# zubair-irshad/HunyuanWorld-Mirror

Hardware: AMD Instinct MI355X
Metric: views/sec (higher is better)
Workload: dtype bf16; 1 GPU; 8-view 518x518 bf16, no priors, camera+depth+pointmap+normal heads, 8 views/GPU, full 1.23B-param arch; views_per_gpu=8, global_views=8, parallelism=view-shard x1, collective=none (1 GPU)

## Files before the change

### hunyuanworld-mirror_amd/_lib.py

```python
from __future__ import annotations

import ctypes as C
import os

import torch

_HERE = os.path.dirname(os.path.abspath(__file__))
LIB_PATH = os.environ.get("WM_HIP_LIB") or os.path.join(_HERE, "libwm_hip.so")

WM_DT = {"bf16": 0, "f16": 1, "fp16": 1, "float16": 1, "bfloat16": 0}
EPI_F32, EPI_T16, EPI_GELU_T16, EPI_RESID = 0, 1, 2, 3


class wm_config(C.Structure):
    _fields_ = [
        ("img_size", C.c_int32), ("patch_size", C.c_int32), ("embed_dim", C.c_int32), ("gs_dim", C.c_int32),
        ("enable_cond", C.c_int32), ("enable_cam", C.c_int32), ("enable_pts", C.c_int32), ("enable_depth", C.c_int32),
        ("enable_norm", C.c_int32), ("enable_gs", C.c_int32),
        ("depth", C.c_int32), ("num_heads", C.c_int32), ("mlp_ratio", C.c_int32), ("num_register_tokens", C.c_int32),
        ("intermediate_idxs", C.c_int32 * 4),
        ("rope_freq", C.c_float),
        ("dino_depth", C.c_int32), ("dino_heads", C.c_int32),
        ("cam_trunk_depth", C.c_int32), ("cam_heads", C.c_int32), ("cam_steps", C.c_int32),
        ("dpt_features", C.c_int32),
# ... 2 lines not shown
    ]


_FP = C.c_void_p


class wm_outputs(C.Structure):
    _fields_ = [(n, _FP) for n in (
        "camera_params", "camera_poses", "camera_intrs", "depth", "depth_conf", "pts3d", "pts3d_conf",
        "normals", "normals_conf", "gs_depth", "gs_depth_conf", "splat_means", "splat_quats", "splat_scales",
        "splat_opacities", "splat_sh", "splat_weights")] + [("taps", _FP * 4)]


class wm_raster_options(C.Structure):
    _fields_ = [("antialiased", C.c_int), ("depth_mode", C.c_int), ("eps2d", C.c_float), ("near_plane", C.c_float), ("far_plane", C.c_float),
                ("radius_clip", C.c_float), ("backgrounds", C.c_void_p)]


EXPORTS = [
    "wm_create", "wm_destroy", "wm_last_error", "wm_set_weight", "wm_finalize_weights", "wm_host_resample_pos",
    "wm_workspace_bytes", "wm_reserve", "wm_set_workspace", "wm_missing_name", "wm_share_weights", "wm_forward", "wm_forward_sharded", "wm_rccl_unique_id", "wm_comm_init_rccl",
    "wm_local_group_create", "wm_local_group_destroy", "wm_comm_init_local", "wm_allgather", "wm_profile_enable", "wm_profile_read",
    "wm_op_gemm", "wm_op_gemm_resid_ln", "wm_op_gemm_qkv", "wm_op_attention", "wm_op_layernorm", "wm_op_qkv_post", "wm_op_conv", "wm_op_bilinear",
    "wm_op_linear_f32", "wm_host_to_16", "wm_set_tuning", "wm_op_attention_split", "wm_op_attention_ex", "wm_op_attention_flag_count", "wm_op_gs_splat", "wm_op_conv3x3_up", "wm_depth_to_world", "wm_confidence_mask", "wm_confidence_mask_workspace_bytes", "wm_preprocess_image", "wm_preprocess_image_size",
    "wm_preprocess_image_workspace_bytes", "wm_rasterize_splats", "wm_rasterize_workspace_bytes", "wm_rasterize_splats_backward", "wm_rasterize_backward_workspace_bytes", "wm_prune_gs", "wm_prune_gs_workspace_bytes", "wm_op_up_conv_n32", "wm_op_conv3x3_gemm16", "wm_op_conv_ex", "wm_op_upconv3x3_tap", "wm_op_tconv", "wm_op_upconv_gather",
    "wm_depth_edge", "wm_normals_edge", "wm_point_filter_mask_workspace_bytes", "wm_point_filter_mask",
    "wm_op_im2col", "wm_op_im2col7", "wm_op_dino_tokens", "wm_op_vgt_special", "wm_op_gemm_rowmap", "wm_op_gemm_convt", "wm_op_layernorm_rows",
    "wm_op_bilinear_add", "wm_op_bilinear16", "wm_op_copy2d", "wm_op_small_attention", "wm_op_adaln", "wm_op_cam_update", "wm_op_cam_matrices",
    "wm_op_linear_f32_ex", "wm_op_dpt_tail", "wm_op_up_conv_n32_tail", "wm_op_dpt_tap_front",
    "wm_photometric_loss_workspace_bytes", "wm_photometric_loss_forward_workspace_bytes", "wm_photometric_loss", "wm_photometric_loss_backward",
    "wm_rasterize_backward_workspace_bytes_ex", "wm_rasterize_splats_backward_ex", "wm_rasterize_means2d",
    "wm_rasterize_backward_workspace_bytes_cam", "wm_rasterize_splats_backward_cam",
    "wm_rasterize_splats_sh", "wm_rasterize_backward_workspace_bytes_sh", "wm_rasterize_splats_backward_sh",
    "wm_rasterize_splats_opt", "wm_rasterize_backward_workspace_bytes_opt", "wm_rasterize_splats_backward_opt",
    "wm_densify_accumulate", "wm_densify_plan_workspace_bytes", "wm_densify_plan", "wm_densify_gather",
    "wm_mcmc_inject_noise", "wm_mcmc_partition_workspace_bytes", "wm_mcmc_partition", "wm_mcmc_relocation", "wm_mcmc_scatter", "wm_mcmc_zero_rows",
    "wm_bilagrid_slice", "wm_bilagrid_slice_backward_workspace_bytes", "wm_bilagrid_slice_backward", "wm_bilagrid_tv_workspace_bytes",
    "wm_bilagrid_tv", "wm_bilagrid_tv_backward",
    "wm_appearance_forward", "wm_appearance_backward_workspace_bytes", "wm_appearance_backward",
    "wm_depth_loss_workspace_bytes", "wm_depth_loss", "wm_depth_loss_backward", "wm_project_depth_points",
]

_lib = None


def lib() -> C.CDLL:
    global _lib
# ... 22 lines not shown
    L.wm_missing_name.argtypes = [vp, i32]
    L.wm_missing_name.restype = C.c_char_p
    L.wm_forward.argtypes = [vp, vp, i32, i32, i32, vp, vp, vp, C.POINTER(C.c_int32), C.POINTER(wm_outputs), vp]
    L.wm_forward_sharded.argtypes = [vp, vp, i32, i32, i32, i32, i32, vp, vp, vp, C.POINTER(C.c_int32),
                                     C.POINTER(wm_outputs), vp]
    L.wm_rccl_unique_id.argtypes = [vp]
    L.wm_comm_init_rccl.argtypes = [vp, vp, i32, i32]
    L.wm_local_group_create.argtypes = [i32]
    L.wm_local_group_create.restype = vp
    L.wm_local_group_destroy.argtypes = [vp]
    L.wm_local_group_destroy.restype = None
    L.wm_comm_init_local.argtypes = [vp, vp, i32]
    L.wm_allgather.argtypes = [vp, vp, vp, C.c_size_t, vp]
    L.wm_profile_enable.argtypes = [vp, i32]
    L.wm_profile_read.argtypes = [vp, i32, C.POINTER(C.c_double), C.POINTER(C.c_int64)]
    L.wm_op_gemm.argtypes = [i32, i32, vp, vp, vp, vp, vp, i32, i32, i32, vp]
    L.wm_op_gemm_resid_ln.argtypes = [i32, vp, vp, vp, vp, vp, vp, vp, f32, vp, vp, vp, i32, i32, i32, C.POINTER(i32), vp]
    L.wm_op_gemm_qkv.argtypes = [i32, vp, vp, vp, vp, vp, vp, vp, vp, vp, vp, vp, vp, i32, i32, i32, i32, i32, i32, f32, vp]
    L.wm_op_attention.argtypes = [i32, vp, vp, vp, vp, i32, i32, i32, i32, i32, vp]
    L.wm_op_attention_split.argtypes = [i32, vp, vp, vp, vp, i32, i32, i32, i32, i32, i32, vp, vp, vp]
    L.wm_op_attention_ex.argtypes = [i32, vp, vp, vp, vp, i32, i32, i32, i32, i32, i32, vp, vp, vp, vp]
    L.wm_op_attention_flag_count.argtypes = [i32, i32, i32]
    L.wm_op_attention_flag_count.restype = C.c_size_t
    L.wm_op_layernorm.argtypes = [vp, vp, vp, vp, i32, i32, f32, i32, i32, vp]
    L.wm_op_qkv_post.argtypes = [i32, vp, vp, vp, vp, vp, vp, vp, vp, vp, vp, i32, i32, i32, i32, i32, f32, vp]
    L.wm_op_conv.argtypes = [i32, vp, vp, vp, vp, vp, vp, i32, i32, i32, i32, i32, i32, i32, i32, i32, i32, vp]
    L.wm_op_bilinear.argtypes = [vp, vp, i32, i32, i32, i32, i32, i32, vp]
    L.wm_op_linear_f32.argtypes = [vp, vp, vp, vp, i32, i32, i32, i32, i32, i32, vp]
    L.wm_host_to_16.argtypes = [vp, vp, C.c_size_t, i32]
    L.wm_host_to_16.restype = None
    L.wm_depth_to_world.argtypes = [vp, vp, vp, vp, vp, vp, i32, i32, i32, f32, vp]
    L.wm_depth_to_world.restype = i32
    L.wm_confidence_mask_workspace_bytes.argtypes = [C.c_size_t]
    L.wm_confidence_mask_workspace_bytes.restype = C.c_size_t
    L.wm_confidence_mask.argtypes = [vp, C.c_size_t, f32, vp, vp, C.c_size_t, vp]
    L.wm_confidence_mask.restype = i32
    L.wm_depth_edge.argtypes = [vp, vp, i32, i32, i32, i32, i32, f32, i32, f32, vp, vp]
    L.wm_depth_edge.restype = i32
    L.wm_normals_edge.argtypes = [vp, vp, i32, i32, i32, i32, C.c_double, vp, vp]
    L.wm_normals_edge.restype = i32
    L.wm_point_filter_mask_workspace_bytes.argtypes = [i32, i32, i32]
    L.wm_point_filter_mask_workspace_bytes.restype = C.c_size_t
    L.wm_point_filter_mask.argtypes = [vp, vp, vp, i32, i32, i32, i32, C.c_double, i32, C.c_double, f32, vp, vp, vp, C.c_size_t, vp]
    L.wm_point_filter_mask.restype = i32
    L.wm_op_up_conv_n32.argtypes = [i32, vp, vp, vp, vp, i32, i32, i32, i32, i32, i32, vp, vp, i32, vp, vp]
    L.wm_op_up_conv_n32.restype = i32
# ... 162 lines not shown
```

### hunyuanworld-mirror_amd/csrc/attention.hip

```cpp
#include "wm_common.h"
#include "wm_kernels.h"

namespace {

__device__ __forceinline__ void wm_dma16(const void* g, uint32_t lds_dst) {
  uint32_t keep;
  asm volatile("s_mov_b32 %0, m0\n\ts_mov_b32 m0, %2\n\ts_nop 0\n\tglobal_load_lds_dwordx4 %1, off\n\ts_mov_b32 m0, %0"
               : "=&s"(keep) : "v"(g), "s"(lds_dst) : "memory");
}

constexpr int KVB = 64;
constexpr int TILE_B = KVB * 64 * 2;
constexpr float LOG2E = 1.4426950408889634f;

typedef __attribute__((address_space(3))) s16x4* lds_s16x4p;

typedef __attribute__((ext_vector_type(2))) float f32x2;
typedef __attribute__((ext_vector_type(2))) __bf16 bf16x2;
typedef __attribute__((ext_vector_type(2))) _Float16 f16x2;
__device__ __forceinline__ uint32_t pack2(float a, float b, int T) {
  const f32x2 v = {a, b};
  return T == WM_T_BF16 ? __builtin_bit_cast(uint32_t, __builtin_convertvector(v, bf16x2))
                        : __builtin_bit_cast(uint32_t, __builtin_convertvector(v, f16x2));
}
// ... 559 lines not shown
    M = fmaxf(M, ml.x);
  }
  float L = 0.f;
  float4 o = make_float4(0, 0, 0, 0);
  for (int s = 0; s < p.kv_splits; ++s) {
    const float w = __builtin_amdgcn_exp2f(m[s] - M);
    L += w * l[s];
    const float4 v = *(const float4*)(p.part_o + ((size_t)s * p.q_rows + row) * (p.H * 64) + head * 64 + d4 * 4);
    o.x += w * v.x; o.y += w * v.y; o.z += w * v.z; o.w += w * v.w;
  }
  const float inv = 1.0f / L;
  uint2 u;
  u.x = pack2(o.x * inv, o.y * inv, T);
  u.y = pack2(o.z * inv, o.w * inv, T);
  *(uint2*)((u16*)p.O + (row * p.H + head) * 64 + d4 * 4) = u;
}

template <int T, int NW, int QB, int MINW, int LZ = 1, int STG = 1>
hipError_t launch(const WmAttnArgs& a_in, hipStream_t s, int fast = 0) {
  const bool use_v3 = fast != 0;
  constexpr int QT = NW * 32 * QB;
  WmAttnArgs a = a_in;
  a.only_if = nullptr;
  const int tiles_per_seq = (a.seq_len + QT - 1) / QT;
  const int nseq = a.q_rows / a.seq_len;
  {
    static const int ncu = [] { hipDeviceProp_t pr; int d = 0; (void)hipGetDevice(&d); return hipGetDeviceProperties(&pr, d) == hipSuccess ? pr.multiProcessorCount : 256; }();
    const long slots = (long)ncu * MINW * 4 / NW, blocks = (long)tiles_per_seq * nseq * a.H;
    const int seg_rows = a.kv_chunks > 1 ? a.kv_rows_per_chunk : a.seq_len;
    const int ntiles = (seg_rows + KVB - 1) / KVB * a.kv_chunks;
    int lim = a.part_o && a.part_ml ? (a.max_splits > 0 ? a.max_splits : WM_ATTN_MAX_SPLITS) : 1;
    lim = lim < WM_ATTN_MAX_SPLITS ? lim : WM_ATTN_MAX_SPLITS;
    lim = lim < ntiles / 8 ? lim : (ntiles / 8 > 1 ? ntiles / 8 : 1);
    int best = 1;
    const int forced_splits = wm_tune(WM_TUNE_ATTN_SPLITS, 0);
    const int tail_mode = wm_tune(WM_TUNE_ATTN_TAIL, 1);
    if (a.kv_splits > 0) best = a.kv_splits < lim ? a.kv_splits : lim;
    else if (forced_splits > 0) best = forced_splits < lim ? forced_splits : lim;
    else if (a.kv_chunks > 1 && lim >= 2) best = lim < 4 ? lim : 4;
    if (a.force_partial) best = a_in.kv_splits > 0 ? (a_in.kv_splits < lim ? a_in.kv_splits : lim) : 1;
    a.kv_splits = best;
    a.full_units = 0;
    const long tail = blocks % slots;
    if (!a.force_partial && a_in.kv_splits == 0 && forced_splits <= 0 && lim >= 2 && ntiles >= (use_v3 ? 16 : 64) && blocks > slots && tail > 0 && tail_mode != 0) {
      auto round_cost = [&](long n) { const long rem = n % slots; return (double)(n / slots) + (rem == 0 ? 0.0 : (rem * 2 <= slots && fast != 4) ? 0.73 : 1.0); };
      double best_cost = round_cost(tail);
      int bs = 1;
      for (int S = 2; S <= lim; ++S) {
        const double c = round_cost(tail * S) / S + 0.01 * S;
        if (c < best_cost - 0.05) { best_cost = c; bs = S; }
      }
      if (tail_mode > 1) bs = tail_mode < lim ? tail_mode : lim;
      if (bs > 1) { a.kv_splits = bs; a.full_units = (int)(blocks - tail); }
      else if (best > 1) a.kv_splits = best;
    }
  }
  const int units = tiles_per_seq * nseq * a.H;
  const int nfull = a.kv_splits > 1 ? a.full_units : units;
  dim3 grid(nfull + (units - nfull) * a.kv_splits), block(NW * 64);
  if (use_v3) {
    hipError_t e = fast == 4 ? wm_launch_attention_v4(a, (int)grid.x, a.unit_flags, s) : wm_launch_attention_v3(a, (int)grid.x, a.unit_flags, s);
    if (e != hipSuccess) return e;
    a.only_if = a.unit_flags;
  }
#ifdef WM_ATTN_TIMING_EXPERIMENT
  const int dbg_skip = wm_tune(WM_TUNE_ATTN_DEBUG_SKIP, 0);
#else
  constexpr int dbg_skip = 0;
#endif
  if (!(use_v3 && (dbg_skip & 1))) hipLaunchKernelGGL((attn_fwd_kernel<T, NW, QB, MINW, LZ, STG>), grid, block, 0, s, a);
  if (a.kv_splits > 1 && !a.force_partial && !(dbg_skip & 2))
    hipLaunchKernelGGL((attn_combine_kernel<T>), dim3((unsigned)((units - nfull) * (QT / 16))), dim3(256), 0, s, a, QT);
  return hipGetLastError();
}

}

hipError_t wm_launch_attention_combine(const WmAttnArgs& a_in, int slots, hipStream_t s) {
  if (a_in.q_rows <= 0) return hipSuccess;
  if (slots < 1 || slots > WM_ATTN_MAX_SPLITS || !a_in.part_o || !a_in.part_ml) return hipErrorInvalidValue;
  constexpr int QT = 256;
  WmAttnArgs a = a_in;
  a.kv_splits = slots;
  a.full_units = 0;
  const int units = ((a.seq_len + QT - 1) / QT) * (a.q_rows / a.seq_len) * a.H;
  if (a.dtype == WM_T_BF16) hipLaunchKernelGGL((attn_combine_kernel<WM_T_BF16>), dim3((unsigned)(units * (QT / 16))), dim3(256), 0, s, a, QT);
  else hipLaunchKernelGGL((attn_combine_kernel<WM_T_F16>), dim3((unsigned)(units * (QT / 16))), dim3(256), 0, s, a, QT);
  return hipGetLastError();
}

int wm_attention_variant(const WmAttnArgs& a) {
  const int forced = wm_tune(WM_TUNE_ATTN_QB, 0);
  const int seg_rows = a.kv_chunks > 1 ? a.kv_rows_per_chunk : a.seq_len;
  const bool fast_ok = a.unit_flags != nullptr && seg_rows >= 512;
  const bool v3ok = a.dtype == WM_T_BF16 && fast_ok;
  int qb = forced ? forced : 8;
  if (!forced && a.kv_chunks == 1 && a.seq_len <= 2048) qb = (a.dtype == WM_T_BF16 && a.q_rows / a.seq_len >= 16) ? 7 : 4;
  if ((qb == 7 && !v3ok) || (qb == 8 && !fast_ok) || qb == 0) qb = (a.kv_chunks == 1 && a.seq_len <= 2048) ? 4 : 3;
  if (a.force_partial && qb != 7 && qb != 8 && qb != 3) qb = forced ? -1 : 3;
  return qb;
}
void wm_attention_geometry(const WmAttnArgs& a, int* unit_rows, int* blocks_per_cu) {
  const int qb = wm_attention_variant(a);
  *unit_rows = qb == 8 ? 512 : qb == 4 || qb == 11 ? 128 : 256;
  *blocks_per_cu = qb == 8 ? 1 : qb == 4 || qb == 11 ? 3 : 2;
}

hipError_t wm_launch_attention(const WmAttnArgs& a, hipStream_t s) {
  if (a.q_rows <= 0) return hipSuccess;
  if (a.seq_len <= 0 || a.q_rows % a.seq_len != 0 || a.kv_chunks < 1) return hipErrorInvalidValue;
  const int qb = wm_attention_variant(a);
  if (qb < 0) return hipErrorInvalidValue;
  const int seg_rows = a.kv_chunks > 1 ? a.kv_rows_per_chunk : a.seq_len;
  if (qb == 7) return launch<WM_T_BF16, 4, 2, 2>(a, s, 3);
  if (qb == 8) {
    if (!a.unit_flags) return hipErrorInvalidValue;
    return a.dtype == WM_T_BF16 ? launch<WM_T_BF16, 8, 2, 2>(a, s, 4) : launch<WM_T_F16, 8, 2, 2>(a, s, 4);
  }
  if (qb == 6) return a.dtype == WM_T_BF16 ? launch_sp<WM_T_BF16, 1>(a, s) : launch_sp<WM_T_F16, 1>(a, s);
  if (qb == 10) return a.dtype == WM_T_BF16 ? launch<WM_T_BF16, 4, 2, 2, 0>(a, s) : launch<WM_T_F16, 4, 2, 2, 0>(a, s);
  if (qb == 11) return a.dtype == WM_T_BF16 ? launch<WM_T_BF16, 4, 1, 3, 0>(a, s) : launch<WM_T_F16, 4, 1, 3, 0>(a, s);
  if (qb == 13) return a.dtype == WM_T_BF16 ? launch<WM_T_BF16, 4, 2, 2, 1, 2>(a, s) : launch<WM_T_F16, 4, 2, 2, 1, 2>(a, s);
  if (qb == 2) return a.dtype == WM_T_BF16 ? launch<WM_T_BF16, 4, 2, 1>(a, s) : launch<WM_T_F16, 4, 2, 1>(a, s);
  if (qb == 3) return a.dtype == WM_T_BF16 ? launch<WM_T_BF16, 4, 2, 2>(a, s) : launch<WM_T_F16, 4, 2, 2>(a, s);
  if (qb == 4) return a.dtype == WM_T_BF16 ? launch<WM_T_BF16, 4, 1, 3>(a, s) : launch<WM_T_F16, 4, 1, 3>(a, s);
  return a.dtype == WM_T_BF16 ? launch<WM_T_BF16, 4, 1, 2>(a, s) : launch<WM_T_F16, 4, 1, 2>(a, s);
}
```

### hunyuanworld-mirror_amd/csrc/wm_kernels.h

```cpp
#pragma once
#include <hip/hip_runtime.h>
#include <stdint.h>
#include <stddef.h>


enum {
  WM_EPI_F32 = 0,
  WM_EPI_T16 = 1,
  WM_EPI_GELU_T16 = 2,
  WM_EPI_RESID = 3,
  WM_EPI_ROWMAP_ADD = 4,
  WM_EPI_CONVT = 5,
  WM_EPI_QKV = 6,
  WM_EPI_CONV = 7,
};

struct WmQkvArgs {
  const float* qkv; void* q; void* k; void* v;
  const float* qn_w; const float* qn_b; const float* kn_w; const float* kn_b;
  const float* rope_cos; const float* rope_sin;
  int M, H, head_stride;
  int tokens_per_view, patch_start, grid_w;
  float inv_tpv, inv_gw;
  float q_scale; int dtype;
// ... 33 lines not shown
struct WmAttnArgs {
  const void* Q; const void* K; const void* V;
  void* O;
  int H;
  int q_rows;
  int seq_len;
  int q_head_stride;
  int kv_head_stride;
  int kv_chunks;
  long long kv_chunk_stride;
  int kv_rows_per_chunk;
  int dtype;
  int kv_splits, max_splits;
  int full_units;
  float* part_o; float* part_ml;
  int* unit_flags;
  const int* only_if;
  int* unit_hint;
  int* unit_stat;
  int force_partial, part_slot0;
};
hipError_t wm_launch_attention_combine(const WmAttnArgs& a, int slots, hipStream_t s);
hipError_t wm_launch_attention(const WmAttnArgs& a, hipStream_t s);
int wm_attention_variant(const WmAttnArgs& a);
void wm_attention_geometry(const WmAttnArgs& a, int* unit_rows, int* blocks_per_cu);
hipError_t wm_launch_attention_v3(const WmAttnArgs& a, int grid, int* flags, hipStream_t s);
hipError_t wm_launch_attention_v4(const WmAttnArgs& a, int grid, int* flags, hipStream_t s);
inline size_t wm_attention_max_blocks(int q_rows, int seq_len, int H) {
  const size_t nseq = (size_t)(q_rows / (seq_len > 0 ? seq_len : 1));
  return ((size_t)(seq_len + 127) / 128 + 1) * nseq * (size_t)H * WM_ATTN_MAX_SPLITS_C;
}
constexpr int WM_ATTN_MAX_SPLITS = 8;
constexpr int WM_ATTN_HINT_TTL = 15;

struct WmLnArgs {
  const float* x; void* y; const float* w; const float* b;
  int D, ld_in, ld_out; float eps;
  int groups, rows_per_group, in_group, in_off, out_group, out_off;
  int out_f32, dtype;
};
hipError_t wm_launch_layernorm(const WmLnArgs& a, hipStream_t s);

hipError_t wm_launch_qkv_post(const WmQkvArgs& a, hipStream_t s);

hipError_t wm_launch_im2col(const float* img, void* out, int N, int C, int H, int W, int ps, int Kpad,
                            int normalize, int dtype, hipStream_t s);
// ... 217 lines not shown
  X(CONV_RS, "conv_rs") \
  X(LIN_MFMA, "lin_mfma") \
  X(CONV_TPX, "conv_tpx") \
  X(ATTN_TAIL, "attn_tail") \
  X(GEMM_GROUP, "gemm_group") \
  X(COMM_OVERLAP, "comm_overlap") \
  X(HEADS_CONC, "heads_concurrent") \
  X(RCU_MID16, "rcu_mid16") \
  X(GEMM_SCHED, "gemm_sched") \
  X(FORCE_GATHER, "force_gather") \
  X(ATTN_OP_POLICY, "attn_op_policy") \
  X(COMM_P2P, "comm_p2p") \
  X(LN_RPW, "ln_rpw") \
  X(LN_FUSE, "ln_fuse") \
  X(HEADS_MAIN, "heads_main") \
  X(CONV_GEMM, "conv_gemm") \
  X(RESID_PREFETCH, "resid_prefetch") \
  X(UP1_GATHER, "up1_gather") \
  X(TCONV, "tconv") \
  X(UP1_COMP, "up1_comp") \
  X(CONV_BM, "conv_bm") \
  X(RASTER_PPL, "raster_ppl") \
  X(TAP_SHARED, "tap_shared") \
  X(ATTN_DEBUG_SKIP, "attn_debug_skip") \
  X(CONV_DBG, "conv_dbg") \
  X(DBG_SPLAT, "dbg_splat")
#define WM_TUNE_ENUM(name_, key_) WM_TUNE_##name_,
enum { WM_TUNE_KEYS(WM_TUNE_ENUM) WM_TUNE_COUNT };
#undef WM_TUNE_ENUM
extern int wm_tuning[WM_TUNE_COUNT];
inline int wm_tune(int key, int dflt) { return wm_tuning[key] < 0 ? dflt : wm_tuning[key]; }
```

### hunyuanworld-mirror_amd/csrc/wm_model.cpp

```cpp
#include <hip/hip_runtime.h>
#include <rccl/rccl.h>
#include <pthread.h>

#include <algorithm>
#include <cmath>
#include <cstdio>
#include <cstdlib>
#include <cstring>
#include <map>
#include <string>
#include <unordered_map>
#include <vector>

#include "../../include/wm_hip.h"
#include "wm_kernels.h"

namespace {

inline int ru(int x, int m) { return (x + m - 1) / m * m; }

inline uint16_t h_f2bf(float f) {
  uint32_t u;
  memcpy(&u, &f, 4);
  if ((u & 0x7fffffffu) > 0x7f800000u) return (uint16_t)((u >> 16) | 0x40);
// ... 917 lines not shown
    ex.ln_stats = B<float>(h, "LN_STATS");
    int* sync = B<int>(h, "LN_SYNC");
    ex.ln_sync = sync; ex.ln_fallback = sync + ((size_t)d.Mx / 16 + 2) * 2;
  };
  {
    WmGemmArgs ex;
    memset(&ex, 0, sizeof(ex));
    WmQkvArgs& a = ex.qkv;
    a.q = Q16; a.k = K16; a.v = V16;
    if (qk_norm) {
      a.qn_w = F(h, p + "attn.q_norm.weight"); a.qn_b = F(h, p + "attn.q_norm.bias");
      a.kn_w = F(h, p + "attn.k_norm.weight"); a.kn_b = F(h, p + "attn.k_norm.bias");
    }
    if (rope) { a.rope_cos = B<float>(h, "rope_cos"); a.rope_sin = B<float>(h, "rope_sin"); }
    a.M = M; a.H = heads; a.head_stride = M; a.tokens_per_view = tokens_per_view; a.patch_start = patch_start; a.grid_w = d.gw;
    a.q_scale = 0.125f * 1.4426950408889634f; a.dtype = dt;
    st = gemm(c, dt, WM_EPI_QKV, A16, D, W16(h, p + "attn.qkv.weight"), D, nullptr, 0, F(h, p + "attn.qkv.bias"), nullptr, M, 3 * D, D, &ex);
    if (st) return st;
  }
  {
    WmAttnArgs a;
    memset(&a, 0, sizeof(a));
    a.Q = Q16; a.O = O16; a.H = heads; a.q_rows = M; a.q_head_stride = M; a.dtype = dt;
    const bool force_gather = wm_tune(WM_TUNE_FORCE_GATHER, 0) > 0;
    a.part_o = B<float>(h, "ATT_PO"); a.part_ml = B<float>(h, "ATT_ML"); a.max_splits = WM_ATTN_MAX_SPLITS;
    a.unit_flags = B<int>(h, "ATT_FLAGS");
    const size_t hint_n = wm_attention_max_blocks((int)d.Mx, d.P < d.Td ? d.P : d.Td, d.heads);
    const int site = c.attn_site++;
    int* const hint0 = B<int>(h, "ATT_HINT") + (size_t)site * 3 * hint_n;
    int* const stat0 = B<int>(h, "ATT_STAT") + (size_t)site * 3;
    a.unit_hint = hint0; a.unit_stat = stat0;
    bool general_only = false;
    if (site * 3 < h->att_stat_n) {
      const int cur = h->att_stat_host[site * 3], delta = cur - h->att_seen[site * 3];
      h->att_seen[site * 3] = cur;
      const long units = (long)((seq_len + 511) / 512) * (M / (seq_len > 0 ? seq_len : 1)) * heads;
      if (delta > 0 && (long)delta * 4 >= units) h->att_general_ttl[site * 3] = WM_ATTN_HINT_TTL;
      if (h->att_general_ttl[site * 3] > 0) { --h->att_general_ttl[site * 3]; general_only = true; }
    }
    const bool sharded = is_global && (d.world > 1 || (force_gather && h->comm.kind != 0));
    const int ntpc = (M + 63) / 64;
    const bool overlap = wm_tune(WM_TUNE_COMM_OVERLAP, 0) != 0;
    bool overlap_ok = sharded && overlap && d.world > 1 && ntpc >= 16;
    if (overlap_ok) {
      WmAttnArgs t = a;
      t.force_partial = 1; t.K = K16; t.V = V16; t.seq_len = M; t.kv_head_stride = M; t.kv_chunks = 1;
      overlap_ok = wm_attention_variant(t) >= 0;
      t.kv_chunks = d.world - 1 > 1 ? d.world - 1 : 2; t.kv_rows_per_chunk = M; t.kv_chunk_stride = (long long)(2 * hsz / 2);
      overlap_ok = overlap_ok && wm_attention_variant(t) >= 0;
    }
    if (overlap_ok) {
      if (!h->cstream) {
        LCHK(c, hipStreamCreateWithFlags(&h->cstream, hipStreamNonBlocking));
        LCHK(c, hipEventCreateWithFlags(&h->cfork, hipEventDisableTiming));
        LCHK(c, hipEventCreateWithFlags(&h->cjoin, hipEventDisableTiming));
      }
      char* KVG = B<char>(h, "KVG");
      const int rank = h->comm.rank, world = d.world;
      LCHK(c, hipEventRecord(h->cfork, c.s));
      static const int ncu = [] { hipDeviceProp_t pr; int dv = 0; (void)hipGetDevice(&dv); return hipGetDeviceProperties(&pr, dv) == hipSuccess ? pr.multiProcessorCount : 256; }();
      auto pick = [&](int chunks, int smax) {
        WmAttnArgs g = a;
        g.force_partial = 1; g.seq_len = M; g.kv_head_stride = M;
// ... 885 lines not shown
  }
  return wm_launch_attention(a, (hipStream_t)stream) == hipSuccess ? WM_OK : WM_ERR_HIP;
}
extern "C" wm_status wm_op_attention_ex(int dtype, const void* Q, const void* K, const void* V, void* O, int H, int q_rows, int seq_len,
                                        int kv_chunks, int kv_rows_per_chunk, int kv_splits, float* part_o, float* part_ml, int* unit_flags,
                                        void* stream) {
  WmAttnArgs a;
  memset(&a, 0, sizeof(a));
  a.Q = Q; a.K = K; a.V = V; a.O = O; a.H = H; a.q_rows = q_rows; a.seq_len = seq_len; a.q_head_stride = q_rows;
  a.kv_chunks = kv_chunks; a.dtype = dtype; a.kv_splits = kv_splits; a.max_splits = WM_ATTN_MAX_SPLITS; a.part_o = part_o; a.part_ml = part_ml;
  a.unit_flags = unit_flags;
  if (unit_flags) {
    const size_t nb = wm_attention_max_blocks(q_rows, seq_len, H);
    a.unit_hint = unit_flags + nb;
    a.unit_stat = unit_flags + 2 * nb;
    const bool policy = wm_tune(WM_TUNE_ATTN_OP_POLICY, 0) == 1;
    static int* mirror = nullptr;
    static const int* key = nullptr;
    static int seen = 0, ttl = 0;
    if (!mirror && hipHostMalloc((void**)&mirror, 4, hipHostMallocDefault) != hipSuccess) return WM_ERR_HIP;
    if (key != unit_flags) { key = unit_flags; seen = 0; ttl = 0; *mirror = 0; }
    const int cur = *mirror, delta = cur - seen;
    seen = cur;
    const long units = (long)((seq_len + 511) / 512) * (q_rows / (seq_len > 0 ? seq_len : 1)) * H;
    if (delta < 0) ttl = 0;
    else if (delta > 0 && (long)delta * 4 >= units) ttl = WM_ATTN_HINT_TTL;
    const bool general_only = policy && ttl > 0;
    if (general_only) --ttl;
    int* stat = a.unit_stat;
    if (general_only) { a.unit_flags = nullptr; a.unit_hint = nullptr; a.unit_stat = nullptr; }
    if (kv_chunks > 1) {
      a.kv_head_stride = kv_rows_per_chunk; a.kv_rows_per_chunk = kv_rows_per_chunk; a.kv_chunk_stride = (long long)H * kv_rows_per_chunk * 64;
    } else {
      a.kv_head_stride = q_rows;
    }
    if (wm_launch_attention(a, (hipStream_t)stream) != hipSuccess) return WM_ERR_HIP;
    return hipMemcpyAsync(mirror, stat, 4, hipMemcpyDeviceToHost, (hipStream_t)stream) == hipSuccess ? WM_OK : WM_ERR_HIP;
  }
  if (kv_chunks > 1) {
    a.kv_head_stride = kv_rows_per_chunk; a.kv_rows_per_chunk = kv_rows_per_chunk; a.kv_chunk_stride = (long long)H * kv_rows_per_chunk * 64;
  } else {
    a.kv_head_stride = q_rows;
  }
  return wm_launch_attention(a, (hipStream_t)stream) == hipSuccess ? WM_OK : WM_ERR_HIP;
}
extern "C" size_t wm_op_attention_flag_count(int q_rows, int seq_len, int H) { return 2 * wm_attention_max_blocks(q_rows, seq_len, H) + 4; }
extern "C" wm_status wm_op_up_conv_n32(int dtype, const float* x, const void* w16, const float* bias, float* y, int N, int Hs, int Ws, int Hi,
                                       int Wi, int Cin, const float* addx, const float* addy, int relu_out, void* up16, void* stream) {
  hipStream_t s = (hipStream_t)stream;
  if (Cin % 64 || !up16) return WM_ERR_INVALID;
  const size_t n16 = (size_t)N * Hi * Wi * Cin;
  uint16_t* zero = (uint16_t*)up16 + ((n16 + 7) & ~(size_t)7);
  if (hipMemsetAsync(zero, 0, 16, s) != hipSuccess) return WM_ERR_HIP;
  if (wm_launch_bilinear16(x, up16, N, Hs, Ws, Hi, Wi, Cin, addx, addy, dtype, s) != hipSuccess) return WM_ERR_HIP;
  WmConvN32Args a;
  memset(&a, 0, sizeof(a));
  a.x = (const uint16_t*)up16; a.w = (const uint16_t*)w16; a.bias = bias; a.y = y; a.zero = zero;
  a.N = N; a.H = Hi; a.W = Wi; a.Cin = Cin; a.relu_out = relu_out; a.dtype = dtype;
  return wm_launch_conv3x3_n32_in16(a, s) == hipSuccess ? WM_OK : WM_ERR_HIP;
}
extern "C" wm_status wm_op_gs_splat(const float* gp, const float* img, const float* depth, const float* cam, float* means, float* quats,
                                    float* scales, float* opac, float* sh, float* wts, int N, int H, int W, void* stream) {
  return wm_launch_gs_splat(gp, img, depth, cam, means, quats, scales, opac, sh, wts, N, H, W, (hipStream_t)stream) == hipSuccess ? WM_OK : WM_ERR_HIP;
}
extern "C" size_t wm_prune_gs_workspace_bytes(size_t n) { return wm_prune_workspace_bytes(n); }
extern "C" wm_status wm_prune_gs(const float* means, const float* quats, const float* scales, const float* opacities, const float* sh,
                                 const float* weights, int n, float voxel_size, float* out_means, float* out_quats, float* out_scales,
                                 float* out_opacities, float* out_sh, int* n_voxels, void* workspace, size_t workspace_bytes, void* stream) {
  if (n < 0 || !(voxel_size > 0.f) || !n_voxels) return WM_ERR_INVALID;
// ... 781 lines not shown
```

### include/wm_hip.h

```cpp
#ifndef WM_HIP_H
#define WM_HIP_H
#include <stddef.h>
#include <stdint.h>

#ifdef __cplusplus
extern "C" {
#endif

typedef struct wm_handle wm_handle;

typedef enum { WM_OK = 0, WM_ERR_INVALID = 1, WM_ERR_HIP = 2, WM_ERR_STATE = 3, WM_ERR_COMM = 4 } wm_status;
typedef enum { WM_DT_BF16 = 0, WM_DT_F16 = 1 } wm_dtype;

typedef struct {
  int32_t img_size, patch_size, embed_dim, gs_dim;
  int32_t enable_cond, enable_cam, enable_pts, enable_depth, enable_norm, enable_gs;
  int32_t depth, num_heads, mlp_ratio, num_register_tokens;
  int32_t intermediate_idxs[4];
  float rope_freq;
  int32_t dino_depth, dino_heads;
  int32_t cam_trunk_depth, cam_heads, cam_steps;
  int32_t dpt_features;
  int32_t dpt_out_channels[4];
  int32_t backbone_dtype;
// ... 47 lines not shown
void wm_local_group_destroy(wm_local_group* g);
wm_status wm_comm_init_local(wm_handle* h, wm_local_group* g, int rank);
wm_status wm_allgather(wm_handle* h, const void* send, void* recv, size_t bytes_per_rank, void* stream);

wm_status wm_profile_enable(wm_handle* h, int on);
wm_status wm_profile_read(wm_handle* h, int kind, double* total_ms, int64_t* launches);

wm_status wm_op_gemm(int dtype, int epi, const void* A, const void* W, void* C, const float* bias, const float* gamma,
                     int M, int N, int K, void* stream);
wm_status wm_op_gemm_qkv(int dtype, const void* A, const void* W, const float* bias, void* q, void* k, void* v, const float* qn_w,
                         const float* qn_b, const float* kn_w, const float* kn_b, const float* rope_cos, const float* rope_sin, int M,
                         int H, int K, int tokens_per_view, int patch_start, int grid_w, float q_scale, void* stream);
wm_status wm_op_gemm_resid_ln(int dtype, const void* A, const void* W, float* X, const float* bias, const float* gamma, const float* ln_w,
                              const float* ln_b, float ln_eps, void* ln_out, float* stats, int* sync, int M, int N, int K, int* fused_out,
                              void* stream);
wm_status wm_op_attention(int dtype, const void* Q, const void* K, const void* V, void* O, int H, int q_rows, int seq_len,
                          int kv_chunks, int kv_rows_per_chunk, void* stream);
wm_status wm_op_attention_split(int dtype, const void* Q, const void* K, const void* V, void* O, int H, int q_rows, int seq_len,
                                int kv_chunks, int kv_rows_per_chunk, int kv_splits, float* part_o, float* part_ml, void* stream);
wm_status wm_op_attention_ex(int dtype, const void* Q, const void* K, const void* V, void* O, int H, int q_rows, int seq_len,
                             int kv_chunks, int kv_rows_per_chunk, int kv_splits, float* part_o, float* part_ml, int* unit_flags,
                             void* stream);
size_t wm_op_attention_flag_count(int q_rows, int seq_len, int H);
wm_status wm_op_gs_splat(const float* gp, const float* img, const float* depth, const float* cam, float* means, float* quats,
                         float* scales, float* opac, float* sh, float* wts, int N, int H, int W, void* stream);
wm_status wm_op_layernorm(const float* x, void* y, const float* w, const float* b, int rows, int D, float eps, int out_f32,
                          int dtype, void* stream);
wm_status wm_op_qkv_post(int dtype, const float* qkv, void* q, void* k, void* v, const float* qn_w, const float* qn_b,
                         const float* kn_w, const float* kn_b, const float* rope_cos, const float* rope_sin, int M, int H,
                         int tokens_per_view, int patch_start, int grid_w, float q_scale, void* stream);
wm_status wm_op_conv(int dtype, const float* x, const void* w16, const float* bias, const float* resid, const float* resid2,
                     float* y, int N, int Hi, int Wi, int Cin, int Cout, int ksize, int stride, int pad, int relu_in,
                     int resid_relu, void* stream);
wm_status wm_op_conv3x3_up(int dtype, const float* x, const void* w16, const float* bias, float* y, int N, int Hs, int Ws, int Hi, int Wi,
                           int Cin, int Cout, const float* addx, const float* addy, void* stream);
wm_status wm_op_bilinear(const float* in, float* out, int N, int Hi, int Wi, int Ho, int Wo, int C, void* stream);
wm_status wm_op_linear_f32(const float* X, const float* W, const float* b, float* Y, int M, int N, int K, int ldx, int pre_act,
                           int post_act, void* stream);

wm_status wm_op_im2col(int dtype, const float* img, void* out, int N, int C, int H, int W, int ps, int Kpad, int normalize, void* stream);
wm_status wm_op_im2col7(int dtype, const float* img, void* out, int N, int H, int W, int Kpad, void* stream);
wm_status wm_op_dino_tokens(const float* patch, const float* cls, const float* reg, const float* pos, float* X, int N, int hw, int R, int D,
                            void* stream);
wm_status wm_op_vgt_special(float* X, const float* cam_tok, const float* reg_tok, const float* pose_tok, const float* ray_tok, int N, int P,
                            int R, int D, int cond, int first_view_global, void* stream);
wm_status wm_op_gemm_rowmap(int dtype, const void* A, const void* W, void* C, const float* bias, const float* add, int M, int N, int K,
// ... 218 lines not shown
```

Baseline: 164.2 views/s.

## Centralize attention launch planning and use fast variant for short sequences

Moves attention variant, grid, split and combine sizing into one planning function that the launcher, geometry query and hint-TTL logic all share, and exposes it through a new C entry point. It adds an 'attn_short' heuristic, on by default, that selects the bf16 recompute fast variant for seq_len at most 2048 even when fewer than 16 sequences are present, provided there are enough KV tiles and units relative to CU count. Tail KV-splitting is now accepted only when an estimated cost model says the saved tile time exceeds the combine overhead. The hint-unit count now uses the real unit rows instead of a hardcoded 512. The added risk is that the heuristic picks the fast variant or rejects splits in cases where the simple rule did better.

After: 165.5 views/s, median of 6. About the same (+0.8%).

```diff
diff --git a/hunyuanworld-mirror_amd/_lib.py b/hunyuanworld-mirror_amd/_lib.py
--- a/hunyuanworld-mirror_amd/_lib.py
+++ b/hunyuanworld-mirror_amd/_lib.py
@@ -48,7 +48,7 @@
     "wm_workspace_bytes", "wm_reserve", "wm_set_workspace", "wm_missing_name", "wm_share_weights", "wm_forward", "wm_forward_sharded", "wm_rccl_unique_id", "wm_comm_init_rccl",
     "wm_local_group_create", "wm_local_group_destroy", "wm_comm_init_local", "wm_allgather", "wm_profile_enable", "wm_profile_read",
     "wm_op_gemm", "wm_op_gemm_resid_ln", "wm_op_gemm_qkv", "wm_op_attention", "wm_op_layernorm", "wm_op_qkv_post", "wm_op_conv", "wm_op_bilinear",
-    "wm_op_linear_f32", "wm_host_to_16", "wm_set_tuning", "wm_op_attention_split", "wm_op_attention_ex", "wm_op_attention_flag_count", "wm_op_gs_splat", "wm_op_conv3x3_up", "wm_depth_to_world", "wm_confidence_mask", "wm_confidence_mask_workspace_bytes", "wm_preprocess_image", "wm_preprocess_image_size",
+    "wm_op_linear_f32", "wm_host_to_16", "wm_set_tuning", "wm_op_attention_split", "wm_op_attention_ex", "wm_op_attention_flag_count", "wm_op_attention_plan", "wm_op_gs_splat", "wm_op_conv3x3_up", "wm_depth_to_world", "wm_confidence_mask", "wm_confidence_mask_workspace_bytes", "wm_preprocess_image", "wm_preprocess_image_size",
     "wm_preprocess_image_workspace_bytes", "wm_rasterize_splats", "wm_rasterize_workspace_bytes", "wm_rasterize_splats_backward", "wm_rasterize_backward_workspace_bytes", "wm_prune_gs", "wm_prune_gs_workspace_bytes", "wm_op_up_conv_n32", "wm_op_conv3x3_gemm16", "wm_op_conv_ex", "wm_op_upconv3x3_tap", "wm_op_tconv", "wm_op_upconv_gather",
     "wm_depth_edge", "wm_normals_edge", "wm_point_filter_mask_workspace_bytes", "wm_point_filter_mask",
     "wm_op_im2col", "wm_op_im2col7", "wm_op_dino_tokens", "wm_op_vgt_special", "wm_op_gemm_rowmap", "wm_op_gemm_convt", "wm_op_layernorm_rows",
@@ -117,6 +117,7 @@
     L.wm_op_attention_ex.argtypes = [i32, vp, vp, vp, vp, i32, i32, i32, i32, i32, i32, vp, vp, vp, vp]
     L.wm_op_attention_flag_count.argtypes = [i32, i32, i32]
     L.wm_op_attention_flag_count.restype = C.c_size_t
+    L.wm_op_attention_plan.argtypes = [i32] * 12 + [C.POINTER(i32)]
     L.wm_op_layernorm.argtypes = [vp, vp, vp, vp, i32, i32, f32, i32, i32, vp]
     L.wm_op_qkv_post.argtypes = [i32, vp, vp, vp, vp, vp, vp, vp, vp, vp, vp, i32, i32, i32, i32, i32, f32, vp]
     L.wm_op_conv.argtypes = [i32, vp, vp, vp, vp, vp, vp, i32, i32, i32, i32, i32, i32, i32, i32, i32, i32, vp]
diff --git a/hunyuanworld-mirror_amd/csrc/attention.hip b/hunyuanworld-mirror_amd/csrc/attention.hip
--- a/hunyuanworld-mirror_amd/csrc/attention.hip
+++ b/hunyuanworld-mirror_amd/csrc/attention.hip
@@ -605,11 +605,81 @@
   constexpr int QT = NW * 32 * QB;
   WmAttnArgs a = a_in;
   a.only_if = nullptr;
+  const WmAttnPlan pl = wm_attention_plan(a_in, wm_attention_cu_count());
+  if (pl.variant < 0 || pl.unit_rows != QT || pl.blocks_per_cu != MINW * 4 / NW || pl.recompute != (use_v3 ? 1 : 0)) return hipErrorInvalidValue;
+  a.kv_splits = pl.kv_splits;
+  a.full_units = pl.full_units;
+  dim3 grid((unsigned)pl.grid), block(NW * 64);
+  if (use_v3) {
+    hipError_t e = fast == 4 ? wm_launch_attention_v4(a, (int)grid.x, a.unit_flags, s) : wm_launch_attention_v3(a, (int)grid.x, a.unit_flags, s);
+    if (e != hipSuccess) return e;
+    a.only_if = a.unit_flags;
+  }
+#ifdef WM_ATTN_TIMING_EXPERIMENT
+  const int dbg_skip = wm_tune(WM_TUNE_ATTN_DEBUG_SKIP, 0);
+#else
+  constexpr int dbg_skip = 0;
+#endif
+  if (!(use_v3 && (dbg_skip & 1))) hipLaunchKernelGGL((attn_fwd_kernel<T, NW, QB, MINW, LZ, STG>), grid, block, 0, s, a);
+  if (a.kv_splits > 1 && !a.force_partial && !(dbg_skip & 2))
+    hipLaunchKernelGGL((attn_combine_kernel<T>), dim3((unsigned)pl.combine_grid), dim3(256), 0, s, a, QT);
+  return hipGetLastError();
+}
+
+}
+
+hipError_t wm_launch_attention_combine(const WmAttnArgs& a_in, int slots, hipStream_t s) {
+  if (a_in.q_rows <= 0) return hipSuccess;
+  if (slots < 1 || slots > WM_ATTN_MAX_SPLITS || !a_in.part_o || !a_in.part_ml) return hipErrorInvalidValue;
+  constexpr int QT = 256;
+  WmAttnArgs a = a_in;
+  a.kv_splits = slots;
+  a.full_units = 0;
+  const int units = ((a.seq_len + QT - 1) / QT) * (a.q_rows / a.seq_len) * a.H;
+  if (a.dtype == WM_T_BF16) hipLaunchKernelGGL((attn_combine_kernel<WM_T_BF16>), dim3((unsigned)(units * (QT / 16))), dim3(256), 0, s, a, QT);
+  else hipLaunchKernelGGL((attn_combine_kernel<WM_T_F16>), dim3((unsigned)(units * (QT / 16))), dim3(256), 0, s, a, QT);
+  return hipGetLastError();
+}
+
+static int plan_variant(const WmAttnArgs& a, int n_cu) {
+  const int forced = wm_tune(WM_TUNE_ATTN_QB, 0);
+  const int seg_rows = a.kv_chunks > 1 ? a.kv_rows_per_chunk : a.seq_len;
+  const bool fast_ok = a.unit_flags != nullptr && seg_rows >= 512;
+  const bool v3ok = a.dtype == WM_T_BF16 && fast_ok;
+  int qb = forced ? forced : 8;
+  if (!forced && a.kv_chunks == 1 && a.seq_len <= 2048) {
+    const int nseq = a.q_rows / a.seq_len;
+    bool fast = nseq >= 16;
+    if (!fast && wm_tune(WM_TUNE_ATTN_SHORT, 1) != 0)
+      fast = (a.seq_len + KVB - 1) / KVB >= 20 && (long)((a.seq_len + 255) / 256) * nseq * a.H > 2L * n_cu;
+    qb = (a.dtype == WM_T_BF16 && fast) ? 7 : 4;
+  }
+  if ((qb == 7 && !v3ok) || (qb == 8 && !fast_ok) || qb == 0) qb = (a.kv_chunks == 1 && a.seq_len <= 2048) ? 4 : 3;
+  if (a.force_partial && qb != 7 && qb != 8 && qb != 3) qb = forced ? -1 : 3;
+  return qb;
+}
+constexpr double WM_ATTN_COMBINE_US = 10.0, WM_ATTN_COMBINE_US_PER_MB = 0.2, WM_ATTN_TILE_US = 2.0;
+
+WmAttnPlan wm_attention_plan(const WmAttnArgs& a_in, int n_cu) {
+  WmAttnPlan pl = {};
+  pl.variant = -1;
+  if (a_in.seq_len <= 0 || a_in.q_rows < 0 || a_in.q_rows % a_in.seq_len != 0 || a_in.kv_chunks < 1 || a_in.H < 1) return pl;
+  if (n_cu < 1) n_cu = 256;
+  const int qb = plan_variant(a_in, n_cu);
+  if (qb < 0) return pl;
+  const bool rows256 = qb == 7 || qb == 3 || qb == 10 || qb == 13 || qb == 6 || qb == 2;
+  const int QT = qb == 8 ? 512 : rows256 ? 256 : 128;
+  const int per_cu = qb == 8 || qb == 2 ? 1 : qb == 4 || qb == 11 ? 3 : 2;
+  const int fast = qb == 7 ? 3 : qb == 8 ? 4 : 0;
+  WmAttnArgs a = a_in;
   const int tiles_per_seq = (a.seq_len + QT - 1) / QT;
   const int nseq = a.q_rows / a.seq_len;
+  const int units = tiles_per_seq * nseq * a.H;
+  pl.variant = qb; pl.unit_rows = QT; pl.blocks_per_cu = per_cu; pl.recompute = fast != 0;
+  pl.kv_splits = 1; pl.grid = units;
+  if (qb == 6) return pl;
   {
-    static const int ncu = [] { hipDeviceProp_t pr; int d = 0; (void)hipGetDevice(&d); return hipGetDeviceProperties(&pr, d) == hipSuccess ? pr.multiProcessorCount : 256; }();
-    const long slots = (long)ncu * MINW * 4 / NW, blocks = (long)tiles_per_seq * nseq * a.H;
+    const long slots = (long)n_cu * per_cu, blocks = units;
     const int seg_rows = a.kv_chunks > 1 ? a.kv_rows_per_chunk : a.seq_len;
     const int ntiles = (seg_rows + KVB - 1) / KVB * a.kv_chunks;
     int lim = a.part_o && a.part_ml ? (a.max_splits > 0 ? a.max_splits : WM_ATTN_MAX_SPLITS) : 1;
@@ -625,68 +695,41 @@
     a.kv_splits = best;
     a.full_units = 0;
     const long tail = blocks % slots;
-    if (!a.force_partial && a_in.kv_splits == 0 && forced_splits <= 0 && lim >= 2 && ntiles >= (use_v3 ? 16 : 64) && blocks > slots && tail > 0 && tail_mode != 0) {
+    if (!a.force_partial && a_in.kv_splits == 0 && forced_splits <= 0 && lim >= 2 && ntiles >= (fast != 0 ? 16 : 64) && blocks > slots && tail > 0 && tail_mode != 0) {
       auto round_cost = [&](long n) { const long rem = n % slots; return (double)(n / slots) + (rem == 0 ? 0.0 : (rem * 2 <= slots && fast != 4) ? 0.73 : 1.0); };
+      const bool in_time = a.kv_chunks == 1 && a.seq_len <= 2048 && wm_tune(WM_TUNE_ATTN_SHORT, 1) != 0;
+      auto pays = [&](int S) {
+        const double gain_us = (round_cost(tail) - round_cost(tail * S) / S) * ntiles * WM_ATTN_TILE_US;
+        const double mb = (double)tail * QT * S * (64 * 4 + 8) * 2 * 1e-6;
+        return gain_us > WM_ATTN_COMBINE_US + WM_ATTN_COMBINE_US_PER_MB * mb;
+      };
       double best_cost = round_cost(tail);
       int bs = 1;
       for (int S = 2; S <= lim; ++S) {
         const double c = round_cost(tail * S) / S + 0.01 * S;
-        if (c < best_cost - 0.05) { best_cost = c; bs = S; }
+        if (c < best_cost - 0.05 && (!in_time || pays(S))) { best_cost = c; bs = S; }
       }
       if (tail_mode > 1) bs = tail_mode < lim ? tail_mode : lim;
       if (bs > 1) { a.kv_splits = bs; a.full_units = (int)(blocks - tail); }
       else if (best > 1) a.kv_splits = best;
     }
   }
-  const int units = tiles_per_seq * nseq * a.H;
   const int nfull = a.kv_splits > 1 ? a.full_units : units;
-  dim3 grid(nfull + (units - nfull) * a.kv_splits), block(NW * 64);
-  if (use_v3) {
-    hipError_t e = fast == 4 ? wm_launch_attention_v4(a, (int)grid.x, a.unit_flags, s) : wm_launch_attention_v3(a, (int)grid.x, a.unit_flags, s);
-    if (e != hipSuccess) return e;
-    a.only_if = a.unit_flags;
-  }
-#ifdef WM_ATTN_TIMING_EXPERIMENT
-  const int dbg_skip = wm_tune(WM_TUNE_ATTN_DEBUG_SKIP, 0);
-#else
-  constexpr int dbg_skip = 0;
-#endif
-  if (!(use_v3 && (dbg_skip & 1))) hipLaunchKernelGGL((attn_fwd_kernel<T, NW, QB, MINW, LZ, STG>), grid, block, 0, s, a);
-  if (a.kv_splits > 1 && !a.force_partial && !(dbg_skip & 2))
-    hipLaunchKernelGGL((attn_combine_kernel<T>), dim3((unsigned)((units - nfull) * (QT / 16))), dim3(256), 0, s, a, QT);
-  return hipGetLastError();
-}
-
-}
-
-hipError_t wm_launch_attention_combine(const WmAttnArgs& a_in, int slots, hipStream_t s) {
-  if (a_in.q_rows <= 0) return hipSuccess;
-  if (slots < 1 || slots > WM_ATTN_MAX_SPLITS || !a_in.part_o || !a_in.part_ml) return hipErrorInvalidValue;
-  constexpr int QT = 256;
-  WmAttnArgs a = a_in;
-  a.kv_splits = slots;
-  a.full_units = 0;
-  const int units = ((a.seq_len + QT - 1) / QT) * (a.q_rows / a.seq_len) * a.H;
-  if (a.dtype == WM_T_BF16) hipLaunchKernelGGL((attn_combine_kernel<WM_T_BF16>), dim3((unsigned)(units * (QT / 16))), dim3(256), 0, s, a, QT);
-  else hipLaunchKernelGGL((attn_combine_kernel<WM_T_F16>), dim3((unsigned)(units * (QT / 16))), dim3(256), 0, s, a, QT);
-  return hipGetLastError();
-}
-
-int wm_attention_variant(const WmAttnArgs& a) {
-  const int forced = wm_tune(WM_TUNE_ATTN_QB, 0);
-  const int seg_rows = a.kv_chunks > 1 ? a.kv_rows_per_chunk : a.seq_len;
-  const bool fast_ok = a.unit_flags != nullptr && seg_rows >= 512;
-  const bool v3ok = a.dtype == WM_T_BF16 && fast_ok;
-  int qb = forced ? forced : 8;
-  if (!forced && a.kv_chunks == 1 && a.seq_len <= 2048) qb = (a.dtype == WM_T_BF16 && a.q_rows / a.seq_len >= 16) ? 7 : 4;
-  if ((qb == 7 && !v3ok) || (qb == 8 && !fast_ok) || qb == 0) qb = (a.kv_chunks == 1 && a.seq_len <= 2048) ? 4 : 3;
-  if (a.force_partial && qb != 7 && qb != 8 && qb != 3) qb = forced ? -1 : 3;
-  return qb;
-}
+  pl.kv_splits = a.kv_splits; pl.full_units = a.full_units;
+  pl.grid = nfull + (units - nfull) * a.kv_splits;
+  pl.combine_grid = a.kv_splits > 1 && !a.force_partial ? (units - nfull) * (QT / 16) : 0;
+  return pl;
+}
+
+int wm_attention_cu_count() {
+  static const int ncu = [] { hipDeviceProp_t pr; int d = 0; (void)hipGetDevice(&d); return hipGetDeviceProperties(&pr, d) == hipSuccess ? pr.multiProcessorCount : 256; }();
+  return ncu;
+}
+int wm_attention_variant(const WmAttnArgs& a) { return wm_attention_plan(a, wm_attention_cu_count()).variant; }
 void wm_attention_geometry(const WmAttnArgs& a, int* unit_rows, int* blocks_per_cu) {
-  const int qb = wm_attention_variant(a);
-  *unit_rows = qb == 8 ? 512 : qb == 4 || qb == 11 ? 128 : 256;
-  *blocks_per_cu = qb == 8 ? 1 : qb == 4 || qb == 11 ? 3 : 2;
+  const WmAttnPlan pl = wm_attention_plan(a, wm_attention_cu_count());
+  *unit_rows = pl.variant < 0 ? 256 : pl.unit_rows;
+  *blocks_per_cu = pl.variant < 0 ? 2 : pl.blocks_per_cu;
 }
 
 hipError_t wm_launch_attention(const WmAttnArgs& a, hipStream_t s) {
diff --git a/hunyuanworld-mirror_amd/csrc/wm_kernels.h b/hunyuanworld-mirror_amd/csrc/wm_kernels.h
--- a/hunyuanworld-mirror_amd/csrc/wm_kernels.h
+++ b/hunyuanworld-mirror_amd/csrc/wm_kernels.h
@@ -79,6 +79,18 @@
 };
 hipError_t wm_launch_attention_combine(const WmAttnArgs& a, int slots, hipStream_t s);
 hipError_t wm_launch_attention(const WmAttnArgs& a, hipStream_t s);
+struct WmAttnPlan {
+  int variant;
+  int unit_rows;
+  int blocks_per_cu;
+  int kv_splits;
+  int full_units;
+  int grid;
+  int combine_grid;
+  int recompute;
+};
+WmAttnPlan wm_attention_plan(const WmAttnArgs& a, int n_cu);
+int wm_attention_cu_count();
 int wm_attention_variant(const WmAttnArgs& a);
 void wm_attention_geometry(const WmAttnArgs& a, int* unit_rows, int* blocks_per_cu);
 hipError_t wm_launch_attention_v3(const WmAttnArgs& a, int grid, int* flags, hipStream_t s);
@@ -342,6 +354,7 @@
   X(CONV_BM, "conv_bm") \
   X(RASTER_PPL, "raster_ppl") \
   X(TAP_SHARED, "tap_shared") \
+  X(ATTN_SHORT, "attn_short") \
   X(ATTN_DEBUG_SKIP, "attn_debug_skip") \
   X(CONV_DBG, "conv_dbg") \
   X(DBG_SPLAT, "dbg_splat")
diff --git a/hunyuanworld-mirror_amd/csrc/wm_model.cpp b/hunyuanworld-mirror_amd/csrc/wm_model.cpp
--- a/hunyuanworld-mirror_amd/csrc/wm_model.cpp
+++ b/hunyuanworld-mirror_amd/csrc/wm_model.cpp
@@ -963,7 +963,6 @@
     WmAttnArgs a;
     memset(&a, 0, sizeof(a));
     a.Q = Q16; a.O = O16; a.H = heads; a.q_rows = M; a.q_head_stride = M; a.dtype = dt;
-    const bool force_gather = wm_tune(WM_TUNE_FORCE_GATHER, 0) > 0;
     a.part_o = B<float>(h, "ATT_PO"); a.part_ml = B<float>(h, "ATT_ML"); a.max_splits = WM_ATTN_MAX_SPLITS;
     a.unit_flags = B<int>(h, "ATT_FLAGS");
     const size_t hint_n = wm_attention_max_blocks((int)d.Mx, d.P < d.Td ? d.P : d.Td, d.heads);
@@ -972,14 +971,19 @@
     int* const stat0 = B<int>(h, "ATT_STAT") + (size_t)site * 3;
     a.unit_hint = hint0; a.unit_stat = stat0;
     bool general_only = false;
+    const bool force_gather = wm_tune(WM_TUNE_FORCE_GATHER, 0) > 0;
+    const bool sharded = is_global && (d.world > 1 || (force_gather && h->comm.kind != 0));
     if (site * 3 < h->att_stat_n) {
       const int cur = h->att_stat_host[site * 3], delta = cur - h->att_seen[site * 3];
       h->att_seen[site * 3] = cur;
-      const long units = (long)((seq_len + 511) / 512) * (M / (seq_len > 0 ? seq_len : 1)) * heads;
+      WmAttnArgs t = a;
+      t.seq_len = sharded ? M : seq_len; t.kv_chunks = sharded ? d.world : 1; t.kv_rows_per_chunk = sharded ? M : 0;
+      int unit_rows = 512, per_cu = 1;
+      wm_attention_geometry(t, &unit_rows, &per_cu);
+      const long units = (long)((t.seq_len + unit_rows - 1) / unit_rows) * (M / (t.seq_len > 0 ? t.seq_len : 1)) * heads;
       if (delta > 0 && (long)delta * 4 >= units) h->att_general_ttl[site * 3] = WM_ATTN_HINT_TTL;
       if (h->att_general_ttl[site * 3] > 0) { --h->att_general_ttl[site * 3]; general_only = true; }
     }
-    const bool sharded = is_global && (d.world > 1 || (force_gather && h->comm.kind != 0));
     const int ntpc = (M + 63) / 64;
     const bool overlap = wm_tune(WM_TUNE_COMM_OVERLAP, 0) != 0;
     bool overlap_ok = sharded && overlap && d.world > 1 && ntpc >= 16;
@@ -1911,7 +1915,10 @@
     if (key != unit_flags) { key = unit_flags; seen = 0; ttl = 0; *mirror = 0; }
     const int cur = *mirror, delta = cur - seen;
     seen = cur;
-    const long units = (long)((seq_len + 511) / 512) * (q_rows / (seq_len > 0 ? seq_len : 1)) * H;
+    a.kv_rows_per_chunk = kv_chunks > 1 ? kv_rows_per_chunk : 0;
+    int unit_rows = 512, per_cu = 1;
+    wm_attention_geometry(a, &unit_rows, &per_cu);
+    const long units = (long)((seq_len + unit_rows - 1) / unit_rows) * (q_rows / (seq_len > 0 ? seq_len : 1)) * H;
     if (delta < 0) ttl = 0;
     else if (delta > 0 && (long)delta * 4 >= units) ttl = WM_ATTN_HINT_TTL;
     const bool general_only = policy && ttl > 0;
@@ -1934,6 +1941,28 @@
   return wm_launch_attention(a, (hipStream_t)stream) == hipSuccess ? WM_OK : WM_ERR_HIP;
 }
 extern "C" size_t wm_op_attention_flag_count(int q_rows, int seq_len, int H) { return 2 * wm_attention_max_blocks(q_rows, seq_len, H) + 4; }
+extern "C" wm_status wm_op_attention_plan(int dtype, int H, int q_rows, int seq_len, int kv_chunks, int kv_rows_per_chunk, int kv_splits,
+                                          int max_splits, int have_partials, int have_flags, int force_partial, int n_cu, int* out) {
+  if (!out || n_cu < 1) return WM_ERR_INVALID;
+  static float some_partials;
+  static int some_flags;
+  WmAttnArgs a;
+  memset(&a, 0, sizeof(a));
+  a.H = H; a.q_rows = q_rows; a.seq_len = seq_len; a.q_head_stride = q_rows; a.kv_chunks = kv_chunks; a.dtype = dtype;
+  a.kv_splits = kv_splits; a.max_splits = max_splits > 0 ? max_splits : WM_ATTN_MAX_SPLITS; a.force_partial = force_partial;
+  if (have_partials) { a.part_o = &some_partials; a.part_ml = &some_partials; }
+  if (have_flags) a.unit_flags = &some_flags;
+  if (kv_chunks > 1) {
+    a.kv_head_stride = kv_rows_per_chunk; a.kv_rows_per_chunk = kv_rows_per_chunk; a.kv_chunk_stride = (long long)H * kv_rows_per_chunk * 64;
+  } else {
+    a.kv_head_stride = q_rows;
+  }
+  const WmAttnPlan pl = wm_attention_plan(a, n_cu);
+  if (pl.variant < 0) return WM_ERR_INVALID;
+  out[0] = pl.variant; out[1] = pl.unit_rows; out[2] = pl.blocks_per_cu; out[3] = pl.kv_splits; out[4] = pl.full_units;
+  out[5] = pl.grid; out[6] = pl.combine_grid; out[7] = pl.recompute;
+  return WM_OK;
+}
 extern "C" wm_status wm_op_up_conv_n32(int dtype, const float* x, const void* w16, const float* bias, float* y, int N, int Hs, int Ws, int Hi,
                                        int Wi, int Cin, const float* addx, const float* addy, int relu_out, void* up16, void* stream) {
   hipStream_t s = (hipStream_t)stream;
diff --git a/include/wm_hip.h b/include/wm_hip.h
--- a/include/wm_hip.h
+++ b/include/wm_hip.h
@@ -93,6 +93,8 @@
                              int kv_chunks, int kv_rows_per_chunk, int kv_splits, float* part_o, float* part_ml, int* unit_flags,
                              void* stream);
 size_t wm_op_attention_flag_count(int q_rows, int seq_len, int H);
+wm_status wm_op_attention_plan(int dtype, int H, int q_rows, int seq_len, int kv_chunks, int kv_rows_per_chunk, int kv_splits,
+                               int max_splits, int have_partials, int have_flags, int force_partial, int n_cu, int* out);
 wm_status wm_op_gs_splat(const float* gp, const float* img, const float* depth, const float* cam, float* means, float* quats,
                          float* scales, float* opac, float* sh, float* wts, int N, int H, int W, void* stream);
 wm_status wm_op_layernorm(const float* x, void* y, const float* w, const float* b, int rows, int D, float eps, int out_f32,
```
